# matajoh/fourier_feature_nets

Measured on AMD Instinct MI355X. Metric: rays/sec (train), higher is better.
Workload: dtype f32

## Files before the change

### fourier_feature_nets_amd/csrc/wgrad.hip

```cpp
#include <type_traits>

#include "wgrad_common.h"

namespace ffn {

typedef float f32x2 __attribute__((ext_vector_type(2)));
__device__ __forceinline__ float comp_of(const f32x4& v, int q) { return v[q]; }
__device__ __forceinline__ float comp_of(const f32x2& v, int q) { return v[q]; }
__device__ __forceinline__ float comp_of(float v, int) { return v; }
template <int NF> struct BOperand { typedef f32x4 type; };
template <> struct BOperand<2> { typedef f32x2 type; };
template <> struct BOperand<4> { typedef float type; };

template <int CA, int CB, bool BIAS, int NF = 1>
__device__ __forceinline__ void unit_segment(const ffn_mlp_chain& ch, const ffn_wgrad_unit& unit,
                                             const ffn_wgrad_segment& seg, char* smem,
                                             const float* __restrict__ saved,
                                             const float* __restrict__ dz, int64_t num_blocks,
                                             float* __restrict__ partials) {
    static_assert(NF == 1 || CB == 4, "only a window of one quadrant folds");
    constexpr int NQ = (CA / 4) * (CB / 4);
    constexpr int CBS = CB / NF;
    constexpr int NCH = CA + CBS;
    constexpr int S = 4 * NQ;
    constexpr int NQM = 4 / NF;
    constexpr int kGroupLanes = 32 / NF;
    const int tid = threadIdx.x;
    const int lane = tid & 63;
    const int hh = lane >> 5;
    const int li = lane & 31;
    const int wave = __builtin_amdgcn_readfirstlane(tid >> 6);
    const int qd = wave & (NQ - 1);
    const int part = NQ == 4 ? 0 : (NQ == 2 ? wave >> 1 : wave);
    const int mp = CB == 8 ? qd >> 1 : qd, np = CB == 8 ? (qd & 1) : 0;
    const int qi = li & (kGroupLanes - 1);
    const int fg = li / kGroupLanes;
    const bool a_ok = li < unit.m_quads - 32 * mp;
    const bool b_ok = qi < unit.n_quads - 32 * np;
    const int64_t a_stride = (int64_t)ch.slot_channels[unit.m_slot] * 128;
    const int64_t b_stride = (int64_t)ch.slot_channels[unit.n_slot] * 128;
    const char* a_s = reinterpret_cast<const char*>(dz + ch.slot_offset[unit.m_slot] * num_blocks * 32) +
                      unit.m_cq0 * 512 + seg.blk_begin * a_stride;
    const char* b_s = reinterpret_cast<const char*>(saved + ch.slot_offset[unit.n_slot] * num_blocks * 32) +
                      unit.n_cq0 * 512 + seg.blk_begin * b_stride;
    a_s = uniform_ptr(a_s);
    b_s = uniform_ptr(b_s);
    const int ca_last = (unit.m_quads >> 3) - 1, cb_last = (unit.n_quads >> 3) - 1;
    const int t16 = tid * 16;

    f32x16 acc[4][4];
#pragma unroll
    for (int p = 0; p < 4; ++p)
#pragma unroll
        for (int q = 0; q < 4; ++q)
#pragma unroll
            for (int r = 0; r < 16; ++r) acc[p][q][r] = 0.0f;
    f32x4 bsum = zero4();

    f32x4 R[NCH];
    typedef const f32x4 __attribute__((address_space(1)))* gptr;
#define FFN_REQUEST(j)                                                                         \
    do {                                                                                       \
        gptr chunk = (j) < CA ? (gptr)(a_s + ((j) < ca_last ? (j) : ca_last) * 4096)           \
                              : (gptr)(b_s + ((j) - CA < cb_last ? (j) - CA : cb_last) * 4096);  \
        asm volatile("" : "+s"(chunk));      \
        R[j] = __builtin_nontemporal_load(&chunk[tid]);                                                                     \
    } while (0)
#define FFN_DEPOSIT(cur, j)                                                                    \
    *reinterpret_cast<f32x4*>(smem + ((j) < CA ? image_a(cur) + (j) * 4096                     \
                                               : image_b(cur) + ((j) - CA) * 4096) + t16) = R[j]

#pragma unroll
    for (int j = 0; j < NCH; ++j) FFN_REQUEST(j);
#pragma unroll
    for (int j = 0; j < NCH; ++j) FFN_DEPOSIT(0, j);
    a_s += a_stride;
    b_s += b_stride;
    if (seg.blk_begin + 1 < seg.blk_end) {
#pragma unroll
        for (int j = 0; j < NCH; ++j) FFN_REQUEST(j);
    }
    a_s += a_stride;
    b_s += b_stride;
    asm volatile("s_waitcnt lgkmcnt(0)" ::: "memory");
    __builtin_amdgcn_s_barrier();

    const unsigned x0 = (unsigned)(((hh ^ (li & 15)) << 4) ^ ((part * S) << 5));
    const unsigned x0b = (unsigned)(((hh ^ (qi & 15)) << 4) ^ ((part * S) << 5));
    const unsigned lds0 = (unsigned)(size_t)smem;
    const unsigned a_row = lds0 + image_a(0) + (a_ok ? (32 * mp + li) * 512 : kImageBytes);
    const unsigned b_row = lds0 + image_b(0) + (b_ok ? (32 * np + qi) * 512 : kImageBytes) +
                           (NF > 1 ? fg * (16 / NF) : 0);
    unsigned a_at[S], b_at[S];
#pragma unroll
    for (int i = 0; i < S; ++i) {
        a_at[i] = a_row + (x0 ^ (unsigned)(i << 5));
        b_at[i] = b_row + (x0b ^ (unsigned)(i << 5));
    }
    typedef typename BOperand<NF>::type bvec;
#define FFN_READ_OPERANDS(dst_a, dst_b, idx, tail)                                             \
    do {                                                                                       \
        if constexpr (NF == 1)                                                                 \
            asm volatile("ds_read_b128 %0, %2 offset:%4\n\tds_read_b128 %1, %3 offset:%4" tail \
                         : "=&v"(dst_a), "=&v"(dst_b) : "v"(a_at[idx]), "v"(b_at[idx]), "i"(kToggle) : "memory"); \
        else if constexpr (NF == 2)                                                            \
            asm volatile("ds_read_b128 %0, %2 offset:%4\n\tds_read_b64 %1, %3 offset:%4" tail  \
                         : "=&v"(dst_a), "=&v"(dst_b) : "v"(a_at[idx]), "v"(b_at[idx]), "i"(kToggle) : "memory"); \
        else                                                                                   \
            asm volatile("ds_read_b128 %0, %2 offset:%4\n\tds_read_b32 %1, %3 offset:%4" tail  \
                         : "=&v"(dst_a), "=&v"(dst_b) : "v"(a_at[idx]), "v"(b_at[idx]), "i"(kToggle) : "memory"); \
    } while (0)

    auto block_body = [&](auto cur_tag, bool has1, bool has2) {
        constexpr int CUR = decltype(cur_tag)::value;
        constexpr int kToggle = CUR * kImageStride;
        f32x4 a, a_n;
        bvec b, b_n;
        FFN_READ_OPERANDS(a, b, 0, "\n\ts_waitcnt lgkmcnt(0)");
#pragma unroll
        for (int i = 0; i < S; ++i) {
            constexpr int kLast = S - 1;
            const int in = i + 1 < S ? i + 1 : kLast;
            FFN_READ_OPERANDS(a_n, b_n, in, "");
            __builtin_amdgcn_sched_barrier(0);
            if (BIAS) bsum += a;
#pragma unroll
            for (int p = 0; p < 4; ++p) {
#pragma unroll
                for (int q = 0; q < NQM; ++q)
                    acc[p][q] = __builtin_amdgcn_mfma_f32_32x32x2f32(a[p], comp_of(b, q), acc[p][q], 0, 0, 0);
                if (p == 0) {
                    if (i < S / 4) {
                        if (has1) {
#pragma unroll
                            for (int j = (i * NCH) / (S / 4); j < ((i + 1) * NCH) / (S / 4); ++j)
                                FFN_DEPOSIT(1 - CUR, j);
                        }
                    } else if (i < 3 * S / 4) {
                        if (has2) {
#pragma unroll
                            for (int j = ((i - S / 4) * NCH) / (S / 2); j < ((i - S / 4 + 1) * NCH) / (S / 2); ++j)
                                FFN_REQUEST(j);
                        }
                    }
                }
            }
            __builtin_amdgcn_sched_barrier(0);
            asm volatile("s_waitcnt lgkmcnt(0)" ::: "memory");
            __builtin_amdgcn_sched_barrier(0);
            a = a_n;
            b = b_n;
        }
        a_s += a_stride;
        b_s += b_stride;
        __builtin_amdgcn_s_barrier();
    };

    for (int64_t blk = seg.blk_begin; blk < seg.blk_end; blk += 2) {
        block_body(std::integral_constant<int, 0>{}, blk + 1 < seg.blk_end, blk + 2 < seg.blk_end);
        if (blk + 1 < seg.blk_end)
            block_body(std::integral_constant<int, 1>{}, blk + 2 < seg.blk_end, blk + 3 < seg.blk_end);
    }
#undef FFN_REQUEST
#undef FFN_DEPOSIT
#undef FFN_READ_OPERANDS

    {
        float* out = partials + (int64_t)(seg.slot + wave) * kPartialFloats;
#pragma unroll
        for (int p = 0; p < 4; ++p)
#pragma unroll
            for (int q = 0; q < NQM; ++q)
#pragma unroll
                for (int r = 0; r < 16; ++r)
                    out[((p * 4 + q) * 16 + r) * 64 + lane] = acc[p][q][r];
        reinterpret_cast<f32x4*>(out + 16 * 16 * 64)[lane] = bsum;
    }
}

__global__ void __launch_bounds__(256, 1)
wgrad_unit_kernel(const ffn_mlp_chain ch, const ffn_wgrad_unit* __restrict__ units,
                  const ffn_wgrad_segment* __restrict__ segments,
                  const int32_t* __restrict__ seg_start, const float* __restrict__ saved,
                  const float* __restrict__ dz, const float* __restrict__ d_logits, int64_t n,
                  float* __restrict__ partials) {
    extern __shared__ __attribute__((aligned(16))) char smem[];
    for (int k = threadIdx.x; k < 4 * 128; k += 256)
        reinterpret_cast<float*>(smem + (k >> 7) * kImageStride + kImageBytes)[k & 127] = 0.0f;
    __syncthreads();
    const int64_t num_blocks = (n + 31) / 32;
    const int seg_lo = seg_start[blockIdx.x], seg_hi = seg_start[blockIdx.x + 1];
    for (int si = seg_lo; si < seg_hi; ++si) {
        ffn_wgrad_segment seg = segments[si];
        if (seg.blk_end > num_blocks) seg.blk_end = num_blocks;
        if (seg.blk_end <= seg.blk_begin) {
            float* out = partials + (int64_t)(seg.slot + (threadIdx.x >> 6)) * kPartialFloats;
            for (int e = threadIdx.x & 63; e < kPartialFloats; e += 64) out[e] = 0.0f;
            continue;
        }
        const ffn_wgrad_unit unit = units[seg.job];
        if (unit.kind == 1) {
            head_segment(ch, unit, seg, smem, saved, d_logits, n, num_blocks, partials);
        } else {
            const bool m_wide = unit.m_quads > 32, n_wide = unit.n_quads > 32;
            const int wave = __builtin_amdgcn_readfirstlane(threadIdx.x >> 6);
            const bool bias = unit.want_bias != 0 && (!n_wide || (wave & 1) == 0);
#define FFN_UNIT(CA, CB, NF)                                                                   \
    do {                                                                                       \
        if (bias) unit_segment<CA, CB, true, NF>(ch, unit, seg, smem, saved, dz, num_blocks, partials);  \
        else unit_segment<CA, CB, false, NF>(ch, unit, seg, smem, saved, dz, num_blocks, partials);      \
    } while (0)
            const int fold = ffn_wgrad_fold(unit.n_quads);
            if (m_wide && n_wide) FFN_UNIT(8, 8, 1);
            else if (n_wide) FFN_UNIT(4, 8, 1);
            else if (m_wide) {
                if (fold == 4) FFN_UNIT(8, 4, 4);
                else if (fold == 2) FFN_UNIT(8, 4, 2);
                else FFN_UNIT(8, 4, 1);
            } else {
                if (fold == 4) FFN_UNIT(4, 4, 4);
                else if (fold == 2) FFN_UNIT(4, 4, 2);
                else FFN_UNIT(4, 4, 1);
            }
#undef FFN_UNIT
        }
        __syncthreads();
    }
}

__global__ void __launch_bounds__(256)
wgrad_reduce_kernel(const ffn_reduce_job* __restrict__ rjobs, const float* __restrict__ partials,
                    float* __restrict__ grads) {
    const ffn_reduce_job job = rjobs[blockIdx.y];
    const int elems = job.kind == 0 ? 16 * 16 * 64 : 4 * 16 * 64;
    for (int e = blockIdx.x * blockDim.x + threadIdx.x; e < elems + 256; e += gridDim.x * blockDim.x) {
        float sum = 0.0f;
        if (e < elems) {
            const int lane = e & 63;
            const int r = (e >> 6) & 15;
            const int tile = e >> 10;
            const int hh = lane >> 5, jj = lane & 31;
            const int i = (r & 3) + 8 * (r >> 2) + 4 * hh;
            int row, kint;
            if (job.kind == 0) {
                const int fold = job.n_fold > 1 ? job.n_fold : 1;
                const int group_lanes = 32 / fold, tiles = 4 / fold;
                const int p = tile >> 2, q = tile & 3;
                if (q >= tiles) continue;
                const int quad = jj % group_lanes;
                row = job.m_ch0 + 4 * i + p;
                kint = job.k_base + 4 * (job.n_quad0 + quad) + (jj / group_lanes) * tiles + q;
                if (quad >= job.n_quads) continue;
            } else {
                const int q = e >> 8, chn = (e >> 6) & 3, col_j = lane & 3;
                row = col_j;
                kint = job.k_base + 4 * (job.n_quad0 + q) + chn;
                if ((lane >> 2) != 0 || col_j >= job.lg_n || q >= job.n_quads) continue;
            }
            if (row >= job.rows) continue;
            const int col = job.col_map[kint];
            if (col < 0) continue;
            for (int s = job.slot_begin; s < job.slot_end; s += job.slot_stride) {
                const float* part = partials + (int64_t)s * kPartialFloats + e;
                if (job.kind == 0) {
                    sum += part[0];
                } else {
#pragma unroll
                    for (int b = 0; b < 16; ++b) sum += part[4 * b];
                }
            }
            grads[job.w_grad_off + (int64_t)row * job.ld + col] = sum;
        } else if (job.has_bias) {
            const int b = e - elems;
            if (job.kind == 0) {
                const int i = b >> 2, p = b & 3;
                if (i >= 32) continue;
                for (int s = job.slot_begin; s < job.slot_end; s += job.slot_stride) {
                    const float* strip = partials + (int64_t)s * kPartialFloats + 16 * 16 * 64;
                    sum += strip[i * 4 + p] + strip[(32 + i) * 4 + p];
                }
                const int row = job.m_ch0 + 4 * i + p;
                if (row < job.rows) grads[job.b_grad_off + row] = sum;
            } else {
                if (b >= job.lg_n) continue;
                for (int s = job.slot_begin; s < job.slot_end; s += job.slot_stride) {
                    const float* strip = partials + (int64_t)s * kPartialFloats + 16 * 16 * 64;
#pragma unroll
                    for (int sbk = 0; sbk < 16; ++sbk) sum += strip[4 * sbk + b];
                }
                grads[job.b_grad_off + b] = sum;
            }
        }
    }
}

}

using namespace ffn;

extern "C" int ffn_mlp_wgrad_units(const ffn_mlp_chain* chain, const ffn_wgrad_unit* units,
                                   const ffn_wgrad_segment* segments, const int32_t* seg_start,
                                   int num_groups, const float* saved, const float* dz,
                                   const float* d_logits, int64_t n, float* partials,
                                   void* stream) {
    if (n <= 0 || num_groups <= 0) return fail_arg("ffn_mlp_wgrad_units: shape");
    const size_t lds = kUnitLdsBytes;
    (void)hipFuncSetAttribute(reinterpret_cast<const void*>(&wgrad_unit_kernel),
                              hipFuncAttributeMaxDynamicSharedMemorySize, (int)lds);
    hipLaunchKernelGGL(wgrad_unit_kernel, dim3(num_groups), dim3(256), lds, (hipStream_t)stream,
                       *chain, units, segments, seg_start, saved, dz, d_logits, n, partials);
    return check_launch("ffn_mlp_wgrad_units");
}

extern "C" int ffn_mlp_wgrad_reduce(const ffn_reduce_job* jobs, int num_jobs,
                                    const float* partials, float* grads, void* stream) {
    if (num_jobs <= 0) return fail_arg("ffn_mlp_wgrad_reduce: no jobs");
    hipLaunchKernelGGL(wgrad_reduce_kernel, dim3(66, num_jobs), dim3(256), 0, (hipStream_t)stream,
                       jobs, partials, grads);
    return check_launch("ffn_mlp_wgrad_reduce");
}

extern "C" int64_t ffn_mlp_wgrad_partial_floats(void) { return kPartialFloats; }
```

Measured before the change: 1.527 million.

## Move wgrad block hand-over barrier before last MFMA step and prefetch next image

The per-block workgroup barrier now sits after the second-to-last MFMA step instead of at the end of the block. The last step's LDS operand read pulls step 0 of the other double-buffer image, so the next block starts without an exposed LDS read latency, and the barrier wait overlaps with the final MFMA step. Optional timestamp instrumentation and a compile flag that restores the late hand-over are also added. This relies on all deposits into the other image finishing before step S-2, which a static_assert checks.

```diff
diff --git a/fourier_feature_nets_amd/csrc/wgrad.hip b/fourier_feature_nets_amd/csrc/wgrad.hip
--- a/fourier_feature_nets_amd/csrc/wgrad.hip
+++ b/fourier_feature_nets_amd/csrc/wgrad.hip
@@ -2,7 +2,37 @@
 
 #include "wgrad_common.h"
 
+#ifdef FFN_WGRAD_STAMPS
+__device__ unsigned long long g_dbg[8192];
+__device__ int g_dbg_n;
+#ifndef FFN_STAMP_GROUP
+#define FFN_STAMP_GROUP 121
+#endif
+#define FFN_STAMP_TAKE(t)                                                                      \
+    do { if (dbg_on) asm volatile("s_memtime %0" : "=s"(t) : : "memory"); } while (0)
+#define FFN_STAMP_NOW(t)                                                                       \
+    do { if (dbg_on) asm volatile("s_memtime %0\n\ts_waitcnt lgkmcnt(0)" : "=s"(t) : : "memory"); } while (0)
+#define FFN_STAMP_PUT(tag, t)                                                                  \
+    do {                                                                                       \
+        if (dbg_on) {                                                                          \
+            if (lane == 0 && dbg_n < 8192)                                                     \
+                g_dbg[dbg_n] = ((unsigned long long)(tag) << 56) | ((t) & 0x00ffffffffffffffull);  \
+            ++dbg_n;                                                                           \
+        }                                                                                      \
+    } while (0)
+#else
+#define FFN_STAMP_TAKE(t) do { } while (0)
+#define FFN_STAMP_NOW(t) do { } while (0)
+#define FFN_STAMP_PUT(tag, t) do { } while (0)
+#endif
+
 namespace ffn {
+
+#ifdef FFN_WGRAD_LATE_HANDOVER
+constexpr bool kEarlyHandover = false;
+#else
+constexpr bool kEarlyHandover = true;
+#endif
 
 typedef float f32x2 __attribute__((ext_vector_type(2)));
 __device__ __forceinline__ float comp_of(const f32x4& v, int q) { return v[q]; }
@@ -48,6 +78,18 @@
     const int ca_last = (unit.m_quads >> 3) - 1, cb_last = (unit.n_quads >> 3) - 1;
     const int t16 = tid * 16;
 
+#ifdef FFN_WGRAD_STAMPS
+    const bool dbg_wave = blockIdx.x == FFN_STAMP_GROUP && wave == 0;
+    bool dbg_on = dbg_wave;
+    int dbg_n = 0;
+    if (dbg_wave) dbg_n = __builtin_amdgcn_readfirstlane(*(volatile int*)&g_dbg_n);
+    unsigned long long ts_seg = 0, ts_blk = 0, ts_step = 0, ts_last = 0, ts_pre = 0, ts_post = 0;
+    bool ts_barrier_pending = false;
+    FFN_STAMP_NOW(ts_seg);
+    FFN_STAMP_PUT(1, ts_seg);
+    FFN_STAMP_PUT(11, (unsigned long long)(seg.blk_end - seg.blk_begin));
+#endif
+
     f32x16 acc[4][4];
 #pragma unroll
     for (int p = 0; p < 4; ++p)
@@ -84,6 +126,8 @@
     b_s += b_stride;
     asm volatile("s_waitcnt lgkmcnt(0)" ::: "memory");
     __builtin_amdgcn_s_barrier();
+    FFN_STAMP_NOW(ts_seg);
+    FFN_STAMP_PUT(2, ts_seg);
 
     const unsigned x0 = (unsigned)(((hh ^ (li & 15)) << 4) ^ ((part * S) << 5));
     const unsigned x0b = (unsigned)(((hh ^ (qi & 15)) << 4) ^ ((part * S) << 5));
@@ -98,31 +142,47 @@
         b_at[i] = b_row + (x0b ^ (unsigned)(i << 5));
     }
     typedef typename BOperand<NF>::type bvec;
-#define FFN_READ_OPERANDS(dst_a, dst_b, idx, tail)                                             \
+#define FFN_READ_OPERANDS(dst_a, dst_b, idx, toggle, tail)                                             \
     do {                                                                                       \
         if constexpr (NF == 1)                                                                 \
             asm volatile("ds_read_b128 %0, %2 offset:%4\n\tds_read_b128 %1, %3 offset:%4" tail \
-                         : "=&v"(dst_a), "=&v"(dst_b) : "v"(a_at[idx]), "v"(b_at[idx]), "i"(kToggle) : "memory"); \
+                         : "=&v"(dst_a), "=&v"(dst_b) : "v"(a_at[idx]), "v"(b_at[idx]), "i"(toggle) : "memory"); \
         else if constexpr (NF == 2)                                                            \
             asm volatile("ds_read_b128 %0, %2 offset:%4\n\tds_read_b64 %1, %3 offset:%4" tail  \
-                         : "=&v"(dst_a), "=&v"(dst_b) : "v"(a_at[idx]), "v"(b_at[idx]), "i"(kToggle) : "memory"); \
+                         : "=&v"(dst_a), "=&v"(dst_b) : "v"(a_at[idx]), "v"(b_at[idx]), "i"(toggle) : "memory"); \
         else                                                                                   \
             asm volatile("ds_read_b128 %0, %2 offset:%4\n\tds_read_b32 %1, %3 offset:%4" tail  \
-                         : "=&v"(dst_a), "=&v"(dst_b) : "v"(a_at[idx]), "v"(b_at[idx]), "i"(kToggle) : "memory"); \
+                         : "=&v"(dst_a), "=&v"(dst_b) : "v"(a_at[idx]), "v"(b_at[idx]), "i"(toggle) : "memory"); \
     } while (0)
 
+    f32x4 a;
+    typename BOperand<NF>::type b;
+    if constexpr (kEarlyHandover)
+        FFN_READ_OPERANDS(a, b, 0, 0, "\n\ts_waitcnt lgkmcnt(0)");
     auto block_body = [&](auto cur_tag, bool has1, bool has2) {
         constexpr int CUR = decltype(cur_tag)::value;
         constexpr int kToggle = CUR * kImageStride;
-        f32x4 a, a_n;
-        bvec b, b_n;
-        FFN_READ_OPERANDS(a, b, 0, "\n\ts_waitcnt lgkmcnt(0)");
+        constexpr int kOther = (1 - CUR) * kImageStride;
+        static_assert(S / 4 - 1 <= S - 2, "deposits must end in front of the hand-over barrier");
+        f32x4 a_n;
+        bvec b_n;
+        FFN_STAMP_TAKE(ts_blk);
+        if constexpr (!kEarlyHandover) FFN_READ_OPERANDS(a, b, 0, kToggle, "\n\ts_waitcnt lgkmcnt(0)");
+#ifdef FFN_WGRAD_STAMPS
+        if (!kEarlyHandover) {
+            FFN_STAMP_PUT(3, ts_blk);
+            if (ts_barrier_pending) { FFN_STAMP_PUT(7, ts_pre); FFN_STAMP_PUT(8, ts_post); }
+            ts_barrier_pending = false;
+        }
+#endif
 #pragma unroll
         for (int i = 0; i < S; ++i) {
             constexpr int kLast = S - 1;
-            const int in = i + 1 < S ? i + 1 : kLast;
-            FFN_READ_OPERANDS(a_n, b_n, in, "");
+            if (i + 1 < S) FFN_READ_OPERANDS(a_n, b_n, i + 1, kToggle, "");
+            else if constexpr (kEarlyHandover) FFN_READ_OPERANDS(a_n, b_n, 0, kOther, "");
+            else FFN_READ_OPERANDS(a_n, b_n, kLast, kToggle, "");
             __builtin_amdgcn_sched_barrier(0);
+            FFN_STAMP_TAKE(ts_step);
             if (BIAS) bsum += a;
 #pragma unroll
             for (int p = 0; p < 4; ++p) {
@@ -146,21 +206,52 @@
                 }
             }
             __builtin_amdgcn_sched_barrier(0);
+            if (i == kLast) FFN_STAMP_TAKE(ts_last);
             asm volatile("s_waitcnt lgkmcnt(0)" ::: "memory");
             __builtin_amdgcn_sched_barrier(0);
+#ifdef FFN_WGRAD_STAMPS
+            if (i == 0 && kEarlyHandover) FFN_STAMP_PUT(3, ts_blk);
+            FFN_STAMP_PUT(16 + i, ts_step);
+            if (i == kLast) {
+                FFN_STAMP_PUT(6, ts_last);
+                if (kEarlyHandover) { FFN_STAMP_PUT(7, ts_pre); FFN_STAMP_PUT(8, ts_post); }
+            }
+#endif
+            if (kEarlyHandover && i == S - 2) {
+                FFN_STAMP_TAKE(ts_pre);
+                __builtin_amdgcn_s_barrier();
+                FFN_STAMP_TAKE(ts_post);
+                __builtin_amdgcn_sched_barrier(0);
+            }
             a = a_n;
             b = b_n;
         }
         a_s += a_stride;
         b_s += b_stride;
-        __builtin_amdgcn_s_barrier();
+        if constexpr (!kEarlyHandover) {
+            FFN_STAMP_TAKE(ts_pre);
+            __builtin_amdgcn_s_barrier();
+            FFN_STAMP_TAKE(ts_post);
+#ifdef FFN_WGRAD_STAMPS
+            ts_barrier_pending = dbg_on;
+#endif
+        }
     };
 
     for (int64_t blk = seg.blk_begin; blk < seg.blk_end; blk += 2) {
+#ifdef FFN_WGRAD_STAMPS
+        dbg_on = dbg_wave && (blk - seg.blk_begin < 6 || blk + 3 >= seg.blk_end);
+#endif
         block_body(std::integral_constant<int, 0>{}, blk + 1 < seg.blk_end, blk + 2 < seg.blk_end);
         if (blk + 1 < seg.blk_end)
             block_body(std::integral_constant<int, 1>{}, blk + 2 < seg.blk_end, blk + 3 < seg.blk_end);
     }
+#ifdef FFN_WGRAD_STAMPS
+    dbg_on = dbg_wave;
+    FFN_STAMP_NOW(ts_seg);
+    if (ts_barrier_pending) { FFN_STAMP_PUT(7, ts_pre); FFN_STAMP_PUT(8, ts_post); }
+    FFN_STAMP_PUT(9, ts_seg);
+#endif
 #undef FFN_REQUEST
 #undef FFN_DEPOSIT
 #undef FFN_READ_OPERANDS
@@ -176,6 +267,11 @@
                     out[((p * 4 + q) * 16 + r) * 64 + lane] = acc[p][q][r];
         reinterpret_cast<f32x4*>(out + 16 * 16 * 64)[lane] = bsum;
     }
+#ifdef FFN_WGRAD_STAMPS
+    FFN_STAMP_NOW(ts_seg);
+    FFN_STAMP_PUT(10, ts_seg);
+    if (dbg_wave && lane == 0) *(volatile int*)&g_dbg_n = dbg_n < 8192 ? dbg_n : 8192;
+#endif
 }
 
 __global__ void __launch_bounds__(256, 1)
@@ -321,3 +417,13 @@
 }
 
 extern "C" int64_t ffn_mlp_wgrad_partial_floats(void) { return kPartialFloats; }
+
+#ifdef FFN_WGRAD_STAMPS
+extern "C" int ffn_dbg_read(long long* out, int reset) {
+    int n = 0;
+    (void)hipMemcpyFromSymbol(&n, HIP_SYMBOL(g_dbg_n), sizeof(int));
+    (void)hipMemcpyFromSymbol(out, HIP_SYMBOL(g_dbg), sizeof(long long) * 8192);
+    if (reset) { int z = 0; (void)hipMemcpyToSymbol(HIP_SYMBOL(g_dbg_n), &z, sizeof(int)); }
+    return n;
+}
+#endif
```

Result: no change. 1.535 million, median of 6 (+0.5%).
